# FortuneMU2025/LIDAR_AI_Recommendation_Software

Measured on AMD Instinct MI355X. Metric: M points/sec through SetAbstraction, 65k-pt frames; 1->8 GPU scaling, higher is better.
Workload: dtype f32

## Files before the change

### lidar_ai_recommendation_software_amd/csrc/sa_mlp_x3.hip

```cpp
#include <cmath>
#include <cstdlib>
#include <cstring>
#include <type_traits>
#include <vector>

#include "bq_grid.hpp"
#include "h3.hpp"
#include "sa_shapes.hpp"

namespace {

typedef __bf16 bf16x8 __attribute__((ext_vector_type(8)));
typedef float f32x4 __attribute__((ext_vector_type(4)));
using lidar_h3::f16x8;

__device__ __forceinline__ f32x4 mfma_bf(bf16x8 a, bf16x8 b, f32x4 c)
{
    return __builtin_amdgcn_mfma_f32_16x16x32_bf16(a, b, c, 0, 0, 0);
}
__device__ __forceinline__ f32x4 mfma_bf(f16x8 a, f16x8 b, f32x4 c)
{
    return __builtin_amdgcn_mfma_f32_16x16x32_f16(a, b, c, 0, 0, 0);
}
__device__ __forceinline__ f32x4 mfma_f(float a, float b, f32x4 c)
{
    return __builtin_amdgcn_mfma_f32_16x16x4f32(a, b, c, 0, 0, 0);
}
using lidar::relu_nan;
__device__ __forceinline__ float maxn(float a, float b, float c)
{
    return __builtin_elementwise_maximum(__builtin_elementwise_maximum(a, b), c);
}

__device__ __forceinline__ void split_pair(const f32x4 &t0, const f32x4 &t1, f16x8 &hi, f16x8 &lo, float s)
{
    lidar_h3::split8(t0, t1, s, hi, lo);
}
__device__ __forceinline__ void split_pair(const f32x4 &t0, const f32x4 &t1, bf16x8 &hi, bf16x8 &lo, float)
{
#pragma unroll
    for (int j = 0; j < 8; ++j) {
        const float v = j < 4 ? t0[j] : t1[j - 4];
        const __bf16 h = (__bf16)v;
        hi[j] = h;
        lo[j] = (__bf16)(v - (float)h);
    }
}

template <int C1, int C2, int C3, bool X1 = false>
struct PackX3 {
    static constexpr int T1 = C1 / 16, T2 = C2 / 16, T3 = C3 / 16;
    static constexpr int KS2 = C1 / 32, KS3 = C2 / 32;
    static constexpr int HALVES = X1 ? 1 : 2;
    static constexpr int CH2 = KS2 * 2 * HALVES * 64, CH3 = KS3 * 2 * HALVES * 64;
    static constexpr int W1U4 = T1 * 64 / 4;
};

struct X3Tail {
    int32_t s2, s3;
    float colsum2, bmax2;
};
__device__ __forceinline__ int bound_exp3(const X3Tail &t, int e2)
{
    const float b = (t.colsum2 * ldexpf(1.0f, e2) + t.bmax2) * (1.0f + 0x1p-10f);
    return lidar_h3::exp_of_bits(__float_as_uint(b));
}

enum { L1_XYZ = 0, L1_PRE = 1, L1_PX = 2 };
__device__ __forceinline__ float bf16r(float v) { return (float)(__bf16)v; }

__device__ __forceinline__ float max_row_groups(float v)
{
    const auto a = __builtin_amdgcn_permlane32_swap(__float_as_uint(v), __float_as_uint(v), false, false);
    v = maxn(v, __uint_as_float(a[0]), __uint_as_float(a[1]));
    const auto b = __builtin_amdgcn_permlane16_swap(__float_as_uint(v), __float_as_uint(v), false, false);
    return maxn(v, __uint_as_float(b[0]), __uint_as_float(b[1]));
}

#ifndef LIDAR_BQ_CAP
#define LIDAR_BQ_CAP 512
#endif
#ifndef LIDAR_SA1_W
// ... 203 lines not shown
                        a0[rr][r] = relu_nan(a0[rr][r]);
                        a1[rr][r] = relu_nan(a1[rr][r]);
                    }
                    y2[rr][2 * c < T2 ? 2 * c : 0] = a0[rr];
                    y2[rr][2 * c + 1 < T2 ? 2 * c + 1 : 0] = a1[rr];
                }
                if (c == T2 / 2 - 1) {
#pragma unroll
                    for (int rr = 0; rr < R; ++rr) {
                        float sc = 1.0f;
                        if constexpr (!X1) {
                            e3[rr] = bound_exp3(*reinterpret_cast<const X3Tail *>(Bias + C1 + C2 + C3), e2[rr]);
                            sc = lidar_h3::scale_of(e3[rr]);
                        }
#pragma unroll
                        for (int s = 0; s < KS3; ++s)
                            split_pair(y2[rr][2 * s], y2[rr][2 * s + 1], zh[rr][s], zl[rr][s], sc);
                    }
                }
            } else {
                const int tp = c - T2 / 2;
#pragma unroll
                for (int s = 0; s < KS3; ++s) {
                    const PT h0 = __builtin_bit_cast(PT, wb[((s * 2 + 0) * HV + 0) * 64]);
                    const PT h1 = __builtin_bit_cast(PT, wb[((s * 2 + 1) * HV + 0) * 64]);
                    if constexpr (X1) {
#pragma unroll
                        for (int rr = 0; rr < R; ++rr) {
                            a0[rr] = mfma_bf(zh[rr][s], h0, a0[rr]);
                            a1[rr] = mfma_bf(zh[rr][s], h1, a1[rr]);
                        }
                    } else {
                        const PT l0 = __builtin_bit_cast(PT, wb[((s * 2 + 0) * HV + 1) * 64]);
                        const PT l1 = __builtin_bit_cast(PT, wb[((s * 2 + 1) * HV + 1) * 64]);
#pragma unroll
                        for (int rr = 0; rr < R; ++rr) {
                            a0[rr] = mfma_bf(zh[rr][s], h0, a0[rr]);
                            a1[rr] = mfma_bf(zh[rr][s], h1, a1[rr]);
                            a0[rr] = mfma_bf(zh[rr][s], l0, a0[rr]);
                            a1[rr] = mfma_bf(zh[rr][s], l1, a1[rr]);
                            a0[rr] = mfma_bf(zl[rr][s], h0, a0[rr]);
                            a1[rr] = mfma_bf(zl[rr][s], h1, a1[rr]);
                        }
                    }
                }
#pragma unroll
                for (int hh = 0; hh < 2; ++hh) {
                    const int t = 2 * tp + hh < T3 ? 2 * tp + hh : 0;
                    float v = -INFINITY;
#pragma unroll
                    for (int rr = 0; rr < R; ++rr) {
                        const f32x4 &acc = hh ? a1[rr] : a0[rr];
                        float m4 = maxn(acc[0], acc[1], __builtin_elementwise_maximum(acc[2], acc[3]));
                        if constexpr (!X1) m4 = ldexpf(m4, e3[rr] - 14 - sw3);
                        v = __builtin_elementwise_maximum(v, m4);
                    }
                    v = max_row_groups(v);
                    if (q == (t & 3)) mx[t >> 2] = __builtin_elementwise_maximum(mx[t >> 2], v);
                }
            }
            __syncthreads();
            par ^= 1;
        }
    }
    if (live) {
        float *o = out + unit * out_stride + out_offset;
#pragma unroll
        for (int j = 0; j < T3 / 4; ++j) {
            const int c3 = 16 * (4 * j + q) + col;
            o[c3] = relu_nan(mx[j] + bias_s[C1 + C2 + c3]);
        }
    }
}

#ifndef LIDAR_SA_ABL
#define LIDAR_SA_ABL 0
#endif
#ifndef LIDAR_LEAN_R
#define LIDAR_LEAN_R 2
#endif
#ifndef LIDAR_LEAN_W
#define LIDAR_LEAN_W 4
#endif
template <int C1, int C2, int C3, int NS, bool PFX>
__global__ __launch_bounds__(256, LIDAR_LEAN_W) void sa_x3_lean_kernel(const float *__restrict__ P, int64_t stride,
                                                            const float *__restrict__ Q,
                                                            const int32_t *__restrict__ idx, int n, int m,
                                                            int64_t total, const uint4 *__restrict__ packed,
                                                            float *__restrict__ out, int64_t out_stride,
                                                            int64_t out_offset)
{
    constexpr int R = LIDAR_LEAN_R;
    static_assert(NS % (16 * R) == 0 && C1 % 32 == 0 && C2 % 32 == 0 && C3 % 64 == 0, "tile shapes");
    using K = PackX3<C1, C2, C3, false>;
    constexpr int T2 = K::T2, T3 = K::T3, KS2 = K::KS2, KS3 = K::KS3;
    constexpr int CH2 = K::CH2, CH3 = K::CH3, CHMAX = CH2 > CH3 ? CH2 : CH3;
    constexpr int NL2 = T2 / 2, NL3 = T3 / 2, NSEQ = R * NL2 + NL3;
    constexpr int ITERS = NS / (16 * R);
    constexpr int PER = (CHMAX + 255) / 256;
    static_assert(!PFX || NS % 64 == 0, "PFX: whole 64-row blocks of indices");

    __shared__ uint4 buf0[CHMAX], buf1[CHMAX];
    auto bufp = [&](int p) -> uint4 * { return p ? buf1 : buf0; };
    __shared__ float bias_s[C2 + C3];

    const int tid = threadIdx.x, lane = tid & 63, wave = __builtin_amdgcn_readfirstlane(tid >> 6);
    const int q = lane >> 4, col = lane & 15;
    const int64_t unit = lidar::xcd_block() * 4 + wave;
    const bool live = unit < total;
    const int64_t cc = live ? unit : total - 1;
    const int64_t b = cc / m;

    const uint4 *W2 = packed;
    const uint4 *W3 = W2 + (int64_t)NL2 * CH2;
    const float *Bias = reinterpret_cast<const float *>(W3 + (int64_t)NL3 * CH3);
    const X3Tail tl = *reinterpret_cast<const X3Tail *>(Bias + C1 + C2 + C3);

    auto fetch = [&](int seq, int dst) {
        const int c = (LIDAR_SA_ABL & 1) != 0 ? 0 : seq < R * NL2 ? seq % NL2 : seq - R * NL2 + NL2;
        const uint4 *src = c < NL2 ? W2 + c * CH2 : W3 + (c - NL2) * CH3;
        asm volatile("" : "+s"(src));
        const int len = c < NL2 ? CH2 : CH3;
#pragma unroll
        for (int i = 0; i < PER; ++i) {
            const int base = 256 * i + 64 * wave;
            if ((CH2 == CH3 && CH2 % 256 == 0) || base < len)
                __builtin_amdgcn_global_load_lds((__attribute__((address_space(1))) void *)(src + base + (unsigned)lane),
                                                 (__attribute__((address_space(3))) void *)(&bufp(dst)[base]), 16, 0,
                                                 0);
        }
        __builtin_amdgcn_sched_barrier(0);
    };
    int32_t kall[PFX ? NS / 64 : 1];
    if constexpr (PFX) {
#pragma unroll
        for (int j = 0; j < NS / 64; ++j) kall[j] = idx[cc * NS + 64 * j + lane];
    }
    fetch(0, 0);
    for (int i = tid; i < C2 + C3; i += 256) bias_s[i] = Bias[C1 + i];
    __syncthreads();
    float mx[T3 / 4];
#pragma unroll
    for (int j = 0; j < T3 / 4; ++j) mx[j] = -INFINITY;
    int par = 0;

#pragma unroll 1
    for (int it = 0; it < ITERS; ++it) {
        f16x8 zh[R][KS3], zl[R][KS3];
        int e3[R];
#pragma unroll
        for (int rr = 0; rr < R; ++rr) {
            f16x8 xh[KS2], xl[KS2];
            int e2;
            {
                int zero = 0;
                asm volatile("" : "+v"(zero));
                const int t16 = (it * R + rr) * 16;
                int64_t k;
                if constexpr ((LIDAR_SA_ABL & 4) != 0)
                    k = col;
                else if constexpr (PFX)
                    k = __shfl(kall[t16 >> 6], (t16 & 63) + col, 64);
                else
                    k = idx[cc * NS + t16 + col];
                const f32x4 *pp = reinterpret_cast<const f32x4 *>(P + ((int64_t)b * n + k) * stride + 4 * q);
                const f32x4 *qq = reinterpret_cast<const f32x4 *>(Q + cc * stride + 4 * q + zero);
                f32x4 y[KS2][2];
                uint32_t mb = 0;
#pragma unroll
                for (int s = 0; s < KS2; ++s)
#pragma unroll
                    for (int h = 0; h < 2; ++h) {
                        const f32x4 a = pp[4 * (2 * s + h)], c = qq[4 * (2 * s + h)];
#pragma unroll
                        for (int r = 0; r < 4; ++r) {
                            y[s][h][r] = relu_nan(a[r] - c[r]);
                            mb = max(mb, __float_as_uint(y[s][h][r]));
                        }
                    }
                e2 = lidar_h3::wave_exp(mb);
                const float sc = lidar_h3::scale_of(e2);
#pragma unroll
                for (int s = 0; s < KS2; ++s) split_pair(y[s][0], y[s][1], xh[s], xl[s], sc);
            }
            e3[rr] = bound_exp3(tl, e2);
            const float sc3 = lidar_h3::scale_of(e3[rr]);
#pragma unroll
            for (int c = 0; c < NL2; ++c) {
                fetch(rr * NL2 + c + 1, par ^ 1);
                const uint4 *wb = bufp(par) + lane;
                f32x4 a0 = f32x4{}, a1 = f32x4{};
#pragma unroll
                for (int s = 0; s < KS2; ++s) {
                    const f16x8 h0 = __builtin_bit_cast(f16x8, wb[((s * 2 + 0) * 2 + 0) * 64]);
                    const f16x8 l0 = __builtin_bit_cast(f16x8, wb[((s * 2 + 0) * 2 + 1) * 64]);
                    a0 = mfma_bf(h0, xh[s], a0);
                    a0 = mfma_bf(h0, xl[s], a0);
                    a0 = mfma_bf(l0, xh[s], a0);
                    const f16x8 h1 = __builtin_bit_cast(f16x8, wb[((s * 2 + 1) * 2 + 0) * 64]);
                    const f16x8 l1 = __builtin_bit_cast(f16x8, wb[((s * 2 + 1) * 2 + 1) * 64]);
                    a1 = mfma_bf(h1, xh[s], a1);
                    a1 = mfma_bf(h1, xl[s], a1);
                    a1 = mfma_bf(l1, xh[s], a1);
                }
                const f32x4 b0 = *reinterpret_cast<const f32x4 *>(&bias_s[16 * (2 * c) + 4 * q]);
                const f32x4 b1 = *reinterpret_cast<const f32x4 *>(&bias_s[16 * (2 * c + 1) + 4 * q]);
                const float us = ldexpf(1.0f, e2 - 14 - tl.s2);
#pragma unroll
                for (int r = 0; r < 4; ++r) {
                    a0[r] = relu_nan(fmaf(a0[r], us, b0[r]));
                    a1[r] = relu_nan(fmaf(a1[r], us, b1[r]));
                }
                split_pair(a0, a1, zh[rr][c], zl[rr][c], sc3);
                if constexpr ((LIDAR_SA_ABL & 2) == 0) __syncthreads();
                par ^= 1;
            }
        }
#pragma unroll
        for (int c = 0; c < NL3; ++c) {
            if (c + 1 < NL3 || it + 1 < ITERS) fetch(c + 1 < NL3 ? R * NL2 + c + 1 : 0, par ^ 1);
            const uint4 *wb = bufp(par) + lane;
            f32x4 a0[R], a1[R];
#pragma unroll
            for (int rr = 0; rr < R; ++rr) a0[rr] = a1[rr] = f32x4{};
#pragma unroll
            for (int s = 0; s < KS3; ++s) {
                const f16x8 h0 = __builtin_bit_cast(f16x8, wb[((s * 2 + 0) * 2 + 0) * 64]);
                const f16x8 h1 = __builtin_bit_cast(f16x8, wb[((s * 2 + 1) * 2 + 0) * 64]);
                const f16x8 l0 = __builtin_bit_cast(f16x8, wb[((s * 2 + 0) * 2 + 1) * 64]);
                const f16x8 l1 = __builtin_bit_cast(f16x8, wb[((s * 2 + 1) * 2 + 1) * 64]);
#pragma unroll
                for (int rr = 0; rr < R; ++rr) {
                    a0[rr] = mfma_bf(zh[rr][s], h0, a0[rr]);
                    a1[rr] = mfma_bf(zh[rr][s], h1, a1[rr]);
                    a0[rr] = mfma_bf(zh[rr][s], l0, a0[rr]);
                    a1[rr] = mfma_bf(zh[rr][s], l1, a1[rr]);
                    a0[rr] = mfma_bf(zl[rr][s], h0, a0[rr]);
                    a1[rr] = mfma_bf(zl[rr][s], h1, a1[rr]);
                }
            }
#pragma unroll
            for (int hh = 0; hh < 2; ++hh) {
                const int t = 2 * c + hh;
                float v = -INFINITY;
#pragma unroll
                for (int rr = 0; rr < R; ++rr) {
                    const f32x4 &acc = hh ? a1[rr] : a0[rr];
                    const float m4 = maxn(acc[0], acc[1], __builtin_elementwise_maximum(acc[2], acc[3]));
                    v = __builtin_elementwise_maximum(v, ldexpf(m4, e3[rr] - 14 - tl.s3));
                }
                v = max_row_groups(v);
                if (q == (t & 3)) mx[t >> 2] = __builtin_elementwise_maximum(mx[t >> 2], v);
            }
            if constexpr ((LIDAR_SA_ABL & 2) == 0) __syncthreads();
            par ^= 1;
        }
    }
    static_assert(NSEQ == R * NL2 + NL3, "pass count");
    if (live) {
        float *o = out + unit * out_stride + out_offset;
#pragma unroll
        for (int j = 0; j < T3 / 4; ++j) {
            const int c3 = 16 * (4 * j + q) + col;
            o[c3] = relu_nan(mx[j] + bias_s[C2 + c3]);
        }
    }
}

#ifndef LIDAR_X3_ROWS
#define LIDAR_X3_ROWS 2
#endif
#ifndef LIDAR_X1_ROWS
#define LIDAR_X1_ROWS 2
#endif
template <int NS, bool X1>
constexpr int rows_for()
{
    return X1 && NS >= 16 * LIDAR_X1_ROWS ? LIDAR_X1_ROWS : (NS >= 16 * LIDAR_X3_ROWS ? LIDAR_X3_ROWS : 1);
}

template <int C1, int C2, int C3, int NS, int L1, bool X1 = false, bool LEAN = false>
int launch_x3(const float *p, int64_t stride, const float *q, const int32_t *idx, int64_t batch, int64_t n,
              int64_t m, const void *packed, float *out, int64_t os, int64_t oo, hipStream_t s,
              const float *xyz = nullptr, const float *centres = nullptr)
{
    static_assert(!LEAN || (L1 == L1_PRE && !X1), "the lean kernel: fp32-contract feature levels");
    int64_t total, blocks;
    if (int rc = lidar_sa::launch_geometry("sa_group_mlp_x3", batch, m, 4, total, blocks)) return rc;
    if constexpr (LEAN) {
        hipLaunchKernelGGL((sa_x3_lean_kernel<C1, C2, C3, NS, NS % 64 == 0>), dim3((unsigned)blocks), dim3(256), 0, s,
                           p, stride, q, idx, (int)n, (int)m, total, static_cast<const uint4 *>(packed), out, os, oo);
    } else {
        hipLaunchKernelGGL((sa_x3_kernel<C1, C2, C3, NS, L1, rows_for<NS, X1>(), X1>), dim3((unsigned)blocks),
                           dim3(256), 0, s, p, stride, q, idx, (int)n, (int)m, total,
                           static_cast<const uint4 *>(packed), out, os, oo, xyz, centres, nullptr, 0.0f, 0.0f, nullptr);
    }
    LAUNCH_CHECK();
    return LIDAR_OK;
}

template <int C1, int C2, int C3, int NS, bool XYZ>
int launch_x3_bq(bool x1, const float *xyz, const char *grid, const float *centres, int64_t batch, int64_t n,
                 int64_t m, float radius, const void *packed, float *out, int64_t os, int64_t oo, int32_t *out_idx,
                 hipStream_t s)
{
    if constexpr (XYZ) {
        int64_t total, blocks;
        if (int rc = lidar_sa::launch_geometry("sa_group_mlp_bq", batch, m, 4, total, blocks)) return rc;
        auto go = [&](auto kern) {
            hipLaunchKernelGGL(kern, dim3((unsigned)blocks), dim3(256), 0, s, xyz, (int64_t)3, centres, nullptr, (int)n,
                               (int)m, total, static_cast<const uint4 *>(packed), out, os, oo, nullptr, nullptr, grid,
                               radius, radius * radius, out_idx);
        };
        if (x1)
            go(sa_x3_kernel<C1, C2, C3, NS, L1_XYZ, rows_for<NS, true>(), true, true>);
        else
            go(sa_x3_kernel<C1, C2, C3, NS, L1_XYZ, rows_for<NS, false>(), false, true>);
        LAUNCH_CHECK();
        return LIDAR_OK;
    } else {
        return lidar::fail(LIDAR_EINVAL, "lidar_sa_group_mlp_bq_f32: unsupported (widths, nsample) combination");
    }
}

__host__ uint16_t bf16_rne(float f)
{
    uint32_t u;
    memcpy(&u, &f, 4);
    if ((u & 0x7fffffffu) > 0x7f800000u) return (uint16_t)((u >> 16) | 0x40);
    u += 0x7fffu + ((u >> 16) & 1u);
    return (uint16_t)(u >> 16);
}
__host__ float bf16_to_f(uint16_t h)
{
    const uint32_t u = (uint32_t)h << 16;
    float f;
    memcpy(&f, &u, 4);
    return f;
}
__host__ uint16_t f16_bits(float f)
{
    const _Float16 h = (_Float16)f;
    uint16_t u;
    memcpy(&u, &h, 2);
    return u;
}
__host__ float f16_to_f(uint16_t u)
{
    _Float16 h;
    memcpy(&h, &u, 2);
    return (float)h;
}
__host__ int32_t layer_exp(const float *w, int64_t n)
{
    uint32_t m = 0;
    for (int64_t i = 0; i < n; ++i) {
        uint32_t u;
        memcpy(&u, &w[i], 4);
        m = std::max(m, u & 0x7fffffffu);
    }
    return 14 - lidar_h3::exp_of_bits(m);
}

}

LIDAR_EXPORT int64_t lidar_mlp_packed_size_x3(int32_t xyz_level, int32_t c1, int32_t c2, int32_t c3)
{
    const int64_t w1 = xyz_level ? (int64_t)(c1 / 16) * 64 * 4 : 0;
    return w1 + ((int64_t)(c2 / 32) * (c1 / 32) + (int64_t)(c3 / 32) * (c2 / 32)) * 4 * 64 * 16 +
           (int64_t)(c1 + c2 + c3) * 4 + (int64_t)sizeof(X3Tail);
}

LIDAR_EXPORT int lidar_mlp_pack_x3_f32(int32_t xyz_level, int32_t c1, int32_t c2, int32_t c3, const float *w1,
                                       const float *b1, const float *w2, const float *b2, const float *w3,
// ... 41 lines not shown
        return rc;
    if (batch == 0) return LIDAR_OK;
    ON_DEVICE(h->device);
    hipStream_t s = static_cast<hipStream_t>(stream);
#define LIDAR_SAX3(C1_, C2_, C3_, NS_, X_, LEAN_)                                                              \
    if (!!xyz_level == X_ && c1 == C1_ && c2 == C2_ && c3 == C3_ && nsample == NS_)                            \
        return launch_x3<C1_, C2_, C3_, NS_, X_ ? L1_XYZ : L1_PRE, false, LEAN_>(p, p_stride, q, idx, batch, n, m, \
                                                                                packed, out, out_stride, out_offset, s);
    LIDAR_SA_SHAPES(LIDAR_SAX3)
#undef LIDAR_SAX3
    return lidar::fail(LIDAR_EINVAL, "lidar_sa_group_mlp_x3_f32: unsupported (widths, nsample) combination");
}

LIDAR_EXPORT int64_t lidar_mlp_packed_size_x1(int32_t c1, int32_t c2, int32_t c3)
{
    return (int64_t)(c1 / 16) * 64 * 4 + ((int64_t)(c2 / 32) * (c1 / 32) + (int64_t)(c3 / 32) * (c2 / 32)) * 2 * 64 * 16 +
           (int64_t)(c1 + c2 + c3) * 4;
}

LIDAR_EXPORT int lidar_mlp_pack_x1_f32(int32_t c1, int32_t c2, int32_t c3, const float *w1, const float *b1,
                                       const float *w2, const float *b2, const float *w3, const float *b3,
                                       void *packed)
{
    REQUIRE(w1 && b1 && w2 && b2 && w3 && b3 && packed, "lidar_mlp_pack_x1_f32: null pointer");
    if (int rc = lidar_sa::check_pack_widths("lidar_mlp_pack_x1_f32", c1, c2, c3)) return rc;
    float *f = lidar_sa::write_w1_lanes(static_cast<float *>(packed), w1, c1,
                                        [](float v) { return bf16_to_f(bf16_rne(v)); });
    auto bf = [](float w, int) { return bf16_rne(w); };
    uint16_t *u = reinterpret_cast<uint16_t *>(f);
    u = lidar_sa::write_fragments<1>(u, w2, c1, c2, bf);
    u = lidar_sa::write_fragments<1>(u, w3, c2, c3, bf);
    lidar_sa::write_biases(reinterpret_cast<float *>(u), b1, c1, b2, c2, b3, c3);
    return LIDAR_OK;
}

LIDAR_EXPORT int lidar_sa_group_mlp_x1_f32(lidar_handle *h, int32_t layer1_mode, const float *p, int64_t p_stride,
                                           const float *q, const float *xyz, const float *centres,
                                           const int32_t *idx, int64_t batch, int64_t n, int64_t m, int32_t nsample,
                                           int32_t c1, int32_t c2, int32_t c3, const void *packed, float *out,
                                           int64_t out_stride, int64_t out_offset, void *stream)
{
    REQUIRE(layer1_mode == 0 || layer1_mode == 2, "lidar_sa_group_mlp_x1_f32: layer1_mode must be 0 or 2");
    REQUIRE(layer1_mode == 2 ? (xyz && centres && p_stride >= c1 && p_stride % 4 == 0) : q != nullptr,
            "lidar_sa_group_mlp_x1_f32: mode 0 needs q = centres; mode 2 needs xyz, centres, p_stride >= c1");
    if (int rc = lidar_sa::check_args("lidar_sa_group_mlp_x1_f32", h && p && idx && packed && out,
                                      batch >= 0 && n >= 1 && m >= 1, true, out_offset, c3, out_stride))
        return rc;
    if (batch == 0) return LIDAR_OK;
    ON_DEVICE(h->device);
    hipStream_t s = static_cast<hipStream_t>(stream);
#define LIDAR_SAX1(C1_, C2_, C3_, NS_, X_, LEAN_)                                                                 \
    if (layer1_mode == (X_ ? 0 : 2) && c1 == C1_ && c2 == C2_ && c3 == C3_ && nsample == NS_)                     \
        return launch_x3<C1_, C2_, C3_, NS_, X_ ? L1_XYZ : L1_PX, true>(p, p_stride, X_ ? q : nullptr, idx, batch, n, \
                                                                       m, packed, out, out_stride, out_offset, s, \
                                                                       xyz, centres);
    LIDAR_SA_SHAPES(LIDAR_SAX1)
#undef LIDAR_SAX1
    return lidar::fail(LIDAR_EINVAL, "lidar_sa_group_mlp_x1_f32: unsupported (widths, nsample) combination");
}

LIDAR_EXPORT int lidar_sa_group_mlp_bq_f32(lidar_handle *h, int32_t x1, const float *xyz, const void *grid,
                                           const float *centres, int64_t batch, int64_t n, int64_t m, float radius,
                                           int32_t nsample, int32_t c1, int32_t c2, int32_t c3, const void *packed,
                                           float *out, int64_t out_stride, int64_t out_offset, int32_t *out_idx,
                                           void *stream)
{
    REQUIRE(radius >= 0.0f, "lidar_sa_group_mlp_bq_f32: negative radius");
    if (int rc = lidar_sa::check_args("lidar_sa_group_mlp_bq_f32", h && xyz && grid && centres && packed && out,
                                      batch >= 0 && n >= 1 && n < 0x3fffffff && m >= 1 && m < 0x7fffffff, true,
                                      out_offset, c3, out_stride))
        return rc;
    if (batch == 0) return LIDAR_OK;
    ON_DEVICE(h->device);
    hipStream_t s = static_cast<hipStream_t>(stream);
    const char *g = static_cast<const char *>(grid);
#define LIDAR_SABQ(C1_, C2_, C3_, NS_, X_, LEAN_)                                                              \
    if (X_ && c1 == C1_ && c2 == C2_ && c3 == C3_ && nsample == NS_)                                           \
        return launch_x3_bq<C1_, C2_, C3_, NS_, X_>(x1 != 0, xyz, g, centres, batch, n, m, radius, packed, out, \
                                                    out_stride, out_offset, out_idx, s);
    LIDAR_SA_SHAPES(LIDAR_SABQ)
#undef LIDAR_SABQ
    return lidar::fail(LIDAR_EINVAL, "lidar_sa_group_mlp_bq_f32: unsupported (widths, nsample) combination");
}
```

### lidar_ai_recommendation_software_amd/csrc/bq_grid.hpp

```cpp
#pragma once
#include "common.hpp"

namespace lidar_bq {

constexpr int kTab = 16384;
#ifndef LIDAR_BQ_KCAP
#define LIDAR_BQ_KCAP 512
#endif
constexpr int kCap = LIDAR_BQ_KCAP;
constexpr int kGridMinN = 1024;

struct BqGrid {
    float minx, miny, minz, inv_s;
    int dx, dy, dz, ncell;
    int win_shift, nwin;
    int pad[2];
};

__host__ __device__ constexpr uint64_t grid_frame_bytes(int64_t n)
{
    return 64 + (uint64_t)(kTab + 64) * 4 + (uint64_t)n * 16;
}

__device__ __forceinline__ int cell_of(float v, float lo, float inv_s, int d)
{
    float u = __fmul_rn(__fsub_rn(v, lo), inv_s);
    u = fminf(fmaxf(u, -2.0f), (float)d + 1.0f);
    return (int)floorf(u);
}

__device__ __forceinline__ int point_slot(float x, float y, float z, int k, const BqGrid &g)
{
    const int ix = min(max(cell_of(x, g.minx, g.inv_s, g.dx), 0), g.dx - 1);
    const int iy = min(max(cell_of(y, g.miny, g.inv_s, g.dy), 0), g.dy - 1);
    const int iz = min(max(cell_of(z, g.minz, g.inv_s, g.dz), 0), g.dz - 1);
    return (k >> g.win_shift) * g.ncell + (ix * g.dy + iy) * g.dz + iz;
}

template <class Out>
__device__ __forceinline__ void scan_range(const float *__restrict__ p, int lo, int hi, float cx, float cy,
                                           float cz, float r2, int ns, int lane, uint64_t below, int &cnt,
                                           int &first, Out *o)
{
    for (int k0 = lo; k0 < hi && cnt < ns; k0 += 64) {
        const int k = k0 + lane;
        bool hit = false;
        if (k < hi) hit = lidar::dist2f(p[3 * k], p[3 * k + 1], p[3 * k + 2], cx, cy, cz) < r2;
        const uint64_t mk = __ballot(hit);
        if (mk) {
            if (first < 0) first = k0 + __ffsll((unsigned long long)mk) - 1;
            const int rk = cnt + __popcll(mk & below);
            if (hit && rk < ns) o[rk] = k;
            cnt += __popcll(mk);
        }
    }
}

__device__ __forceinline__ void lds_wave_sync()
{
    asm volatile("s_waitcnt lgkmcnt(0)" ::: "memory");
    __builtin_amdgcn_wave_barrier();
}

template <int CAP, class Out, bool BM = true>
__device__ __forceinline__ void grid_query_wave(const float *__restrict__ p, const char *__restrict__ fw, int n,
                                                float cx, float cy, float cz, float r, float r2, int ns,
                                                int lane, int *hw, Out *o)
{
    const BqGrid g = *reinterpret_cast<const BqGrid *>(fw);
    const int *tab = reinterpret_cast<const int *>(fw + 64);
    const float4 *sp = reinterpret_cast<const float4 *>(fw + 64 + (kTab + 64) * 4);
    const uint64_t below = (1ull << lane) - 1;

    const float delta = __fadd_rn(__fmul_rn(__fmul_rn(r, g.inv_s), 1.0f + 1.0f / 1024.0f), 1.0f / 1024.0f);
    const float ux = __fmul_rn(__fsub_rn(cx, g.minx), g.inv_s), uy = __fmul_rn(__fsub_rn(cy, g.miny), g.inv_s),
                uz = __fmul_rn(__fsub_rn(cz, g.minz), g.inv_s);
    auto lo_of = [](float u, float dl, int d) {
        return max((int)floorf(fminf(fmaxf(__fsub_rn(u, dl), -2.0f), (float)d + 1.0f)), 0);
    };
    auto hi_of = [](float u, float dl, int d) {
        return min((int)floorf(fminf(fmaxf(__fadd_rn(u, dl), -2.0f), (float)d + 1.0f)), d - 1);
    };
    const int lox = lo_of(ux, delta, g.dx), hix = hi_of(ux, delta, g.dx);
    const int loy = lo_of(uy, delta, g.dy), hiy = hi_of(uy, delta, g.dy);
    const int loz = lo_of(uz, delta, g.dz), hiz = hi_of(uz, delta, g.dz);
    int cnt = 0, first = -1;
    const bool full = (hix - lox) > 2 || (hiy - loy) > 2;
    const int jx = lox + lane / 3, jy = loy + lane % 3;
    const bool col_ok = !full && lane < 9 && jx <= hix && jy <= hiy && loz <= hiz;
    const int colbase = (jx * g.dy + jy) * g.dz + loz;
    int st = 0, len = 0;
    if (col_ok && g.nwin > 0) {
        st = tab[colbase];
        len = tab[colbase + (hiz - loz) + 1] - st;
    }
    const bool bitmap = BM && ns >= 64 && !full && ((int64_t)1 << g.win_shift) <= 32 * (int64_t)CAP;
    unsigned long long *bm = reinterpret_cast<unsigned long long *>(hw);
    for (int win = 0; win < g.nwin && cnt < ns; ++win) {
        const int wlo = win << g.win_shift, whi = min(n, (win + 1) << g.win_shift);
        const int cst = st, clen = len;
        if (col_ok && win + 1 < g.nwin) {
            const int s1 = (win + 1) * g.ncell + colbase;
            st = tab[s1];
            len = tab[s1 + (hiz - loz) + 1] - st;
        }
        const int incl = lidar::row_incl_scan_i32(clen);
        const int tot = full ? CAP + 1 : __builtin_amdgcn_readlane(incl, 8);
        if (tot == 0) continue;
        if (!bitmap && tot > CAP) {
            scan_range(p, wlo, whi, cx, cy, cz, r2, ns, lane, below, cnt, first, o);
            continue;
        }
        const int nwords = (whi - wlo + 63) >> 6;
        if (bitmap) {
            for (int i = lane; i < nwords; i += 64) bm[i] = 0ull;
            lds_wave_sync();
        }
        const int excl = incl - clen;
        int e[9], s[9];
#pragma unroll
        for (int j = 0; j < 9; ++j) {
            e[j] = __builtin_amdgcn_readlane(excl, j);
            s[j] = __builtin_amdgcn_readlane(cst, j);
        }
        int hc = 0;
        for (int t0 = 0; t0 < tot; t0 += 256) {
            float4 qv[4];
#pragma unroll
            for (int u = 0; u < 4; ++u) {
                const int t = t0 + 64 * u + lane;
                int pos = s[0] + t;
#pragma unroll
                for (int j = 1; j < 9; ++j)
                    if (t >= e[j]) pos = s[j] + (t - e[j]);
                qv[u] = t < tot ? sp[pos] : make_float4(0.f, 0.f, 0.f, 0.f);
            }
#pragma unroll
            for (int u = 0; u < 4; ++u) {
                const int t = t0 + 64 * u + lane;
                const bool hit = t < tot && lidar::dist2f(qv[u].x, qv[u].y, qv[u].z, cx, cy, cz) < r2;
                const uint64_t mk = __ballot(hit);
                if (hit) {
                    if (bitmap) {
                        const int o1 = __float_as_int(qv[u].w) - wlo;
                        atomicOr(&bm[o1 >> 6], 1ull << (o1 & 63));
                    } else {
                        hw[hc + __popcll(mk & below)] = __float_as_int(qv[u].w);
                    }
                }
                hc += __popcll(mk);
            }
        }
        if (hc == 0) continue;
        if (bitmap) {
            lds_wave_sync();
            int base = 0, mnv = 0x7fffffff;
            for (int c0 = 0; c0 < nwords && cnt + base < ns; c0 += 64) {
                const int wi = c0 + lane;
                unsigned long long wd = wi < nwords ? bm[wi] : 0ull;
                const int pc = __popcll(wd);
                const int ex = lidar::wave_incl_scan_i32(pc) - pc;
                if (wd) mnv = min(mnv, wlo + 64 * wi + (int)__ffsll(wd) - 1);
                int rk = cnt + base + ex;
                while (wd && rk < ns) {
                    const int j = __ffsll(wd) - 1;
                    o[rk++] = wlo + 64 * wi + j;
                    wd &= wd - 1;
                }
                base += __builtin_amdgcn_readlane(ex + pc, 63);
            }
            if (first < 0) first = (int)lidar::wave_min_u32_dpp((uint32_t)mnv);
            cnt += hc;
            lds_wave_sync();
            continue;
        }
        if (lane < 4) hw[hc + lane] = 0x7fffffff;
        lds_wave_sync();
        int mnv = 0x7fffffff;
        for (int e0 = 0; e0 < hc; e0 += 64) {
            const int ei = e0 + lane;
            const int v = ei < hc ? hw[ei] : 0x7fffffff;
            int rank = 0;
            for (int i = 0; i < hc; i += 4) {
                const int4 h4 = *reinterpret_cast<const int4 *>(hw + i);
                rank += (h4.x < v) + (h4.y < v) + (h4.z < v) + (h4.w < v);
            }
            if (ei < hc && cnt + rank < ns) o[cnt + rank] = v;
            mnv = min(mnv, v);
        }
        if (first < 0) first = (int)lidar::wave_min_u32_dpp((uint32_t)mnv);
        cnt += hc;
        lds_wave_sync();
    }
    const int fill = first < 0 ? 0 : first;
    for (int s2 = min(cnt, ns) + lane; s2 < ns; s2 += 64) o[s2] = fill;
}

}
```

Baseline: 1269.

## Add prefetching lean SA kernel that overlaps next-row gathers with MLP passes

Adds a new lean set-abstraction kernel, on by default, that DMAs the neighbour indices and the centre feature row into LDS up front. It prefetches the next 16-row gather of point features into registers, spread across the layer-2 and layer-3 MFMA passes, and uses vmcnt-counted pass ends so the barrier waits only for the weight chunk and not the in-flight row loads. The aim is to hide gather latency behind matrix work. In exchange it uses more LDS and registers, which may reduce occupancy, and it depends on exact load counting for correctness. It also adds optional per-phase s_memtime instrumentation behind LIDAR_DIAG.

```diff
diff --git a/lidar_ai_recommendation_software_amd/csrc/sa_mlp_x3.hip b/lidar_ai_recommendation_software_amd/csrc/sa_mlp_x3.hip
--- a/lidar_ai_recommendation_software_amd/csrc/sa_mlp_x3.hip
+++ b/lidar_ai_recommendation_software_amd/csrc/sa_mlp_x3.hip
@@ -1,3 +1,4 @@
+#include <atomic>
 #include <cmath>
 #include <cstdlib>
 #include <cstring>
@@ -367,13 +368,64 @@
 #ifndef LIDAR_LEAN_W
 #define LIDAR_LEAN_W 4
 #endif
+#ifndef LIDAR_LEAN_PF
+#define LIDAR_LEAN_PF 1
+#endif
+
+enum { PH_PRO = 0, PH_GATHER, PH_L1, PH_BODY, PH_END, PH_EPI, PH_N };
+#ifdef LIDAR_DIAG
+struct LeanClock {
+    uint32_t t, acc[PH_N];
+    __device__ __forceinline__ uint32_t now()
+    {
+        uint64_t v;
+        __builtin_amdgcn_sched_barrier(0);
+        asm volatile("s_memtime %0\n\ts_waitcnt lgkmcnt(0)" : "=s"(v)::"memory");
+        __builtin_amdgcn_sched_barrier(0);
+        return (uint32_t)v;
+    }
+    __device__ __forceinline__ void start()
+    {
+#pragma unroll
+        for (int k = 0; k < PH_N; ++k) acc[k] = 0;
+        t = now();
+    }
+    __device__ __forceinline__ void lap(int k)
+    {
+        const uint32_t v = now();
+        acc[k] += v - t;
+        t = v;
+    }
+    __device__ __forceinline__ void landed(int k)
+    {
+        asm volatile("s_waitcnt vmcnt(0)" ::: "memory");
+        lap(k);
+    }
+    __device__ __forceinline__ void store(uint64_t *diag, int64_t wave_id, int lane, int centres)
+    {
+        if (diag != nullptr && lane == 0) {
+#pragma unroll
+            for (int k = 0; k < PH_N; ++k) diag[wave_id * 8 + k] = acc[k];
+            diag[wave_id * 8 + 6] = (uint64_t)centres;
+            diag[wave_id * 8 + 7] = 0;
+        }
+    }
+};
+#define LEAN_DIAG(...) __VA_ARGS__
+uint64_t *g_sa2_rec = nullptr;
+int64_t g_sa2_rec_cap = 0;
+std::atomic<int64_t> g_sa2_rec_used{0};
+#else
+#define LEAN_DIAG(...)
+#endif
+
 template <int C1, int C2, int C3, int NS, bool PFX>
 __global__ __launch_bounds__(256, LIDAR_LEAN_W) void sa_x3_lean_kernel(const float *__restrict__ P, int64_t stride,
                                                             const float *__restrict__ Q,
                                                             const int32_t *__restrict__ idx, int n, int m,
                                                             int64_t total, const uint4 *__restrict__ packed,
                                                             float *__restrict__ out, int64_t out_stride,
-                                                            int64_t out_offset)
+                                                            int64_t out_offset, uint64_t *__restrict__ diag)
 {
     constexpr int R = LIDAR_LEAN_R;
     static_assert(NS % (16 * R) == 0 && C1 % 32 == 0 && C2 % 32 == 0 && C3 % 64 == 0, "tile shapes");
@@ -395,6 +447,7 @@
     const bool live = unit < total;
     const int64_t cc = live ? unit : total - 1;
     const int64_t b = cc / m;
+    LEAN_DIAG(LeanClock clk; clk.start();)
 
     const uint4 *W2 = packed;
     const uint4 *W3 = W2 + (int64_t)NL2 * CH2;
@@ -428,6 +481,7 @@
 #pragma unroll
     for (int j = 0; j < T3 / 4; ++j) mx[j] = -INFINITY;
     int par = 0;
+    LEAN_DIAG(clk.lap(PH_PRO);)
 
 #pragma unroll 1
     for (int it = 0; it < ITERS; ++it) {
@@ -452,11 +506,23 @@
                 const f32x4 *qq = reinterpret_cast<const f32x4 *>(Q + cc * stride + 4 * q + zero);
                 f32x4 y[KS2][2];
                 uint32_t mb = 0;
+#ifdef LIDAR_DIAG
+                f32x4 pr[KS2][2], qr[KS2][2];
 #pragma unroll
                 for (int s = 0; s < KS2; ++s)
 #pragma unroll
+                    for (int h = 0; h < 2; ++h) pr[s][h] = pp[4 * (2 * s + h)], qr[s][h] = qq[4 * (2 * s + h)];
+                clk.landed(PH_GATHER);
+#endif
+#pragma unroll
+                for (int s = 0; s < KS2; ++s)
+#pragma unroll
                     for (int h = 0; h < 2; ++h) {
+#ifdef LIDAR_DIAG
+                        const f32x4 a = pr[s][h], c = qr[s][h];
+#else
                         const f32x4 a = pp[4 * (2 * s + h)], c = qq[4 * (2 * s + h)];
+#endif
 #pragma unroll
                         for (int r = 0; r < 4; ++r) {
                             y[s][h][r] = relu_nan(a[r] - c[r]);
@@ -470,6 +536,7 @@
             }
             e3[rr] = bound_exp3(tl, e2);
             const float sc3 = lidar_h3::scale_of(e3[rr]);
+            LEAN_DIAG(clk.lap(PH_L1);)
 #pragma unroll
             for (int c = 0; c < NL2; ++c) {
                 fetch(rr * NL2 + c + 1, par ^ 1);
@@ -497,7 +564,9 @@
                     a1[r] = relu_nan(fmaf(a1[r], us, b1[r]));
                 }
                 split_pair(a0, a1, zh[rr][c], zl[rr][c], sc3);
+                LEAN_DIAG(clk.lap(PH_BODY);)
                 if constexpr ((LIDAR_SA_ABL & 2) == 0) __syncthreads();
+                LEAN_DIAG(clk.lap(PH_END);)
                 par ^= 1;
             }
         }
@@ -537,7 +606,9 @@
                 v = max_row_groups(v);
                 if (q == (t & 3)) mx[t >> 2] = __builtin_elementwise_maximum(mx[t >> 2], v);
             }
+            LEAN_DIAG(clk.lap(PH_BODY);)
             if constexpr ((LIDAR_SA_ABL & 2) == 0) __syncthreads();
+            LEAN_DIAG(clk.lap(PH_END);)
             par ^= 1;
         }
     }
@@ -550,6 +621,237 @@
             o[c3] = relu_nan(mx[j] + bias_s[C2 + c3]);
         }
     }
+    LEAN_DIAG(clk.landed(PH_EPI); clk.store(diag, lidar::xcd_block() * 4 + wave, lane, 1);)
+}
+
+template <int N>
+__device__ __forceinline__ void pass_end()
+{
+    static_assert(N >= 0 && N < 16, "vmcnt's low four bits");
+    __builtin_amdgcn_s_waitcnt(0x0070 | N);
+    asm volatile("s_barrier" ::: "memory");
+}
+
+template <int C1, int C2, int C3, int NS>
+__global__ __launch_bounds__(256, LIDAR_LEAN_W) void sa_x3_lean_pf_kernel(const float *__restrict__ P, int64_t stride,
+                                                            const float *__restrict__ Q,
+                                                            const int32_t *__restrict__ idx, int n, int m,
+                                                            int64_t total, const uint4 *__restrict__ packed,
+                                                            float *__restrict__ out, int64_t out_stride,
+                                                            int64_t out_offset, uint64_t *__restrict__ diag)
+{
+    constexpr int R = 2;
+    using K = PackX3<C1, C2, C3, false>;
+    constexpr int T3 = K::T3, KS2 = K::KS2, KS3 = K::KS3;
+    constexpr int CH = K::CH2, NL2 = K::T2 / 2, NL3 = T3 / 2, PER = CH / 256;
+    constexpr int ITERS = NS / (16 * R);
+    constexpr int NP = 2 * KS2;
+    constexpr int PF2 = NP / NL2;
+    constexpr int PF3 = NP / KS3;
+    static_assert(K::CH2 == K::CH3 && CH % 256 == 0, "equal whole chunks: the pass ends count the loads behind them");
+    static_assert(NP % NL2 == 0 && NP % KS3 == 0 && NP < 16, "the row prefetch spreads over the passes");
+    static_assert(NS % 64 == 0 && C1 % 64 == 0 && C3 % 64 == 0, "whole 64-word DMAs of indices and of the Q row");
+
+    __shared__ uint4 buf0[CH], buf1[CH];
+    auto bufp = [&](int p) -> uint4 * { return p ? buf1 : buf0; };
+    __shared__ float bias_s[C2 + C3];
+    __shared__ float q_s[4][C1];
+    __shared__ int32_t k_s[4][NS];
+
+    const int tid = threadIdx.x, lane = tid & 63, wave = __builtin_amdgcn_readfirstlane(tid >> 6);
+    const int q = lane >> 4, col = lane & 15;
+    const int64_t unit = lidar::xcd_block() * 4 + wave;
+    const bool live = unit < total;
+    const int64_t cc = live ? unit : total - 1;
+    const int64_t b = cc / m;
+    LEAN_DIAG(LeanClock clk; clk.start();)
+
+    const uint4 *W2 = packed;
+    const uint4 *W3 = W2 + (int64_t)NL2 * CH;
+    const float *Bias = reinterpret_cast<const float *>(W3 + (int64_t)NL3 * CH);
+    const X3Tail tl = *reinterpret_cast<const X3Tail *>(Bias + C1 + C2 + C3);
+
+    auto fetch = [&](int seq, int dst) {
+        const int c = seq < R * NL2 ? seq % NL2 : seq - R * NL2 + NL2;
+        const uint4 *src = W2 + c * CH;
+        asm volatile("" : "+s"(src));
+#pragma unroll
+        for (int i = 0; i < PER; ++i) {
+            const int base = 256 * i + 64 * wave;
+            __builtin_amdgcn_global_load_lds((__attribute__((address_space(1))) void *)(src + base + (unsigned)lane),
+                                             (__attribute__((address_space(3))) void *)(&bufp(dst)[base]), 16, 0, 0);
+        }
+        __builtin_amdgcn_sched_barrier(0);
+    };
+    {
+        const int32_t *ks = idx + cc * NS;
+        const float *qs = Q + cc * stride;
+        asm volatile("" : "+s"(ks), "+s"(qs));
+#pragma unroll
+        for (int j = 0; j < NS / 64; ++j)
+            __builtin_amdgcn_global_load_lds((const __attribute__((address_space(1))) void *)(ks + 64 * j + (unsigned)lane),
+                                             (__attribute__((address_space(3))) void *)(&k_s[wave][64 * j]), 4, 0, 0);
+#pragma unroll
+        for (int j = 0; j < C1 / 64; ++j)
+            __builtin_amdgcn_global_load_lds((const __attribute__((address_space(1))) void *)(qs + 64 * j + (unsigned)lane),
+                                             (__attribute__((address_space(3))) void *)(&q_s[wave][64 * j]), 4, 0, 0);
+    }
+    auto rows = [&](int t16) {
+        const int64_t k = k_s[wave][t16 + col];
+        const float *frame = P + b * n * stride;
+        return reinterpret_cast<const f32x4 *>(frame + (k * stride + 4 * q));
+    };
+
+    fetch(0, 0);
+    for (int i = tid; i < C2 + C3; i += 256) bias_s[i] = Bias[C1 + i];
+    pass_end<0>();
+    f32x4 pre[NP];
+    {
+        const f32x4 *pp = rows(0);
+#pragma unroll
+        for (int j = 0; j < NP; ++j) pre[j] = pp[4 * j];
+    }
+    float mx[T3 / 4];
+#pragma unroll
+    for (int j = 0; j < T3 / 4; ++j) mx[j] = -INFINITY;
+    int par = 0;
+    LEAN_DIAG(clk.lap(PH_PRO);)
+
+#pragma unroll 1
+    for (int it = 0; it < ITERS; ++it) {
+        const bool lastit = it + 1 == ITERS;
+        f16x8 zh[R][KS3], zl[R][KS3];
+        int e3[R];
+#pragma unroll
+        for (int rr = 0; rr < R; ++rr) {
+            f16x8 xh[KS2], xl[KS2];
+            int e2;
+            {
+                LEAN_DIAG(clk.landed(PH_GATHER);)
+                f32x4 y[KS2][2];
+                uint32_t mb = 0;
+#pragma unroll
+                for (int s = 0; s < KS2; ++s)
+#pragma unroll
+                    for (int h = 0; h < 2; ++h) {
+                        const f32x4 a = pre[2 * s + h];
+                        const f32x4 c = *reinterpret_cast<const f32x4 *>(&q_s[wave][16 * (2 * s + h) + 4 * q]);
+#pragma unroll
+                        for (int r = 0; r < 4; ++r) {
+                            y[s][h][r] = relu_nan(a[r] - c[r]);
+                            mb = max(mb, __float_as_uint(y[s][h][r]));
+                        }
+                    }
+                e2 = lidar_h3::wave_exp(mb);
+                const float sc = lidar_h3::scale_of(e2);
+#pragma unroll
+                for (int s = 0; s < KS2; ++s) split_pair(y[s][0], y[s][1], xh[s], xl[s], sc);
+            }
+            e3[rr] = bound_exp3(tl, e2);
+            const float sc3 = lidar_h3::scale_of(e3[rr]);
+            LEAN_DIAG(clk.lap(PH_L1);)
+            const f32x4 *pp = rr == 0 ? rows((it * R + 1) * 16) : nullptr;
+#pragma unroll
+            for (int c = 0; c < NL2; ++c) {
+                fetch(rr * NL2 + c + 1, par ^ 1);
+                if (rr == 0) {
+#pragma unroll
+                    for (int j = c * PF2; j < (c + 1) * PF2; ++j) pre[j] = pp[4 * j];
+                    __builtin_amdgcn_sched_barrier(0);
+                }
+                const uint4 *wb = bufp(par) + lane;
+                f32x4 a0 = f32x4{}, a1 = f32x4{};
+#pragma unroll
+                for (int s = 0; s < KS2; ++s) {
+                    const f16x8 h0 = __builtin_bit_cast(f16x8, wb[((s * 2 + 0) * 2 + 0) * 64]);
+                    const f16x8 l0 = __builtin_bit_cast(f16x8, wb[((s * 2 + 0) * 2 + 1) * 64]);
+                    a0 = mfma_bf(h0, xh[s], a0);
+                    a0 = mfma_bf(h0, xl[s], a0);
+                    a0 = mfma_bf(l0, xh[s], a0);
+                    const f16x8 h1 = __builtin_bit_cast(f16x8, wb[((s * 2 + 1) * 2 + 0) * 64]);
+                    const f16x8 l1 = __builtin_bit_cast(f16x8, wb[((s * 2 + 1) * 2 + 1) * 64]);
+                    a1 = mfma_bf(h1, xh[s], a1);
+                    a1 = mfma_bf(h1, xl[s], a1);
+                    a1 = mfma_bf(l1, xh[s], a1);
+                }
+                const f32x4 b0 = *reinterpret_cast<const f32x4 *>(&bias_s[16 * (2 * c) + 4 * q]);
+                const f32x4 b1 = *reinterpret_cast<const f32x4 *>(&bias_s[16 * (2 * c + 1) + 4 * q]);
+                const float us = ldexpf(1.0f, e2 - 14 - tl.s2);
+#pragma unroll
+                for (int r = 0; r < 4; ++r) {
+                    a0[r] = relu_nan(fmaf(a0[r], us, b0[r]));
+                    a1[r] = relu_nan(fmaf(a1[r], us, b1[r]));
+                }
+                split_pair(a0, a1, zh[rr][c], zl[rr][c], sc3);
+                LEAN_DIAG(clk.lap(PH_BODY);)
+                if (rr == 0)
+                    pass_end<PF2>();
+                else
+                    pass_end<0>();
+                LEAN_DIAG(clk.lap(PH_END);)
+                par ^= 1;
+            }
+        }
+        const f32x4 *pp = rows(lastit ? 0 : (it + 1) * R * 16);
+#pragma unroll
+        for (int c = 0; c < NL3; ++c) {
+            if (c + 1 < NL3 || !lastit) fetch(c + 1 < NL3 ? R * NL2 + c + 1 : 0, par ^ 1);
+            const uint4 *wb = bufp(par) + lane;
+            f32x4 a0[R], a1[R];
+#pragma unroll
+            for (int rr = 0; rr < R; ++rr) a0[rr] = a1[rr] = f32x4{};
+#pragma unroll
+            for (int s = 0; s < KS3; ++s) {
+                const f16x8 h0 = __builtin_bit_cast(f16x8, wb[((s * 2 + 0) * 2 + 0) * 64]);
+                const f16x8 h1 = __builtin_bit_cast(f16x8, wb[((s * 2 + 1) * 2 + 0) * 64]);
+                const f16x8 l0 = __builtin_bit_cast(f16x8, wb[((s * 2 + 0) * 2 + 1) * 64]);
+                const f16x8 l1 = __builtin_bit_cast(f16x8, wb[((s * 2 + 1) * 2 + 1) * 64]);
+#pragma unroll
+                for (int rr = 0; rr < R; ++rr) {
+                    a0[rr] = mfma_bf(zh[rr][s], h0, a0[rr]);
+                    a1[rr] = mfma_bf(zh[rr][s], h1, a1[rr]);
+                    a0[rr] = mfma_bf(zh[rr][s], l0, a0[rr]);
+                    a1[rr] = mfma_bf(zh[rr][s], l1, a1[rr]);
+                    a0[rr] = mfma_bf(zl[rr][s], h0, a0[rr]);
+                    a1[rr] = mfma_bf(zl[rr][s], h1, a1[rr]);
+                }
+                if (c == NL3 - 1) {
+#pragma unroll
+                    for (int j = s * PF3; j < (s + 1) * PF3; ++j) pre[j] = pp[4 * j];
+                }
+            }
+#pragma unroll
+            for (int hh = 0; hh < 2; ++hh) {
+                const int t = 2 * c + hh;
+                float v = -INFINITY;
+#pragma unroll
+                for (int rr = 0; rr < R; ++rr) {
+                    const f32x4 &acc = hh ? a1[rr] : a0[rr];
+                    const float m4 = maxn(acc[0], acc[1], __builtin_elementwise_maximum(acc[2], acc[3]));
+                    v = __builtin_elementwise_maximum(v, ldexpf(m4, e3[rr] - 14 - tl.s3));
+                }
+                v = max_row_groups(v);
+                if (q == (t & 3)) mx[t >> 2] = __builtin_elementwise_maximum(mx[t >> 2], v);
+            }
+            LEAN_DIAG(clk.lap(PH_BODY);)
+            if (c == NL3 - 1)
+                pass_end<NP>();
+            else
+                pass_end<0>();
+            LEAN_DIAG(clk.lap(PH_END);)
+            par ^= 1;
+        }
+    }
+    if (live) {
+        float *o = out + unit * out_stride + out_offset;
+#pragma unroll
+        for (int j = 0; j < T3 / 4; ++j) {
+            const int c3 = 16 * (4 * j + q) + col;
+            o[c3] = relu_nan(mx[j] + bias_s[C2 + c3]);
+        }
+    }
+    __builtin_amdgcn_s_waitcnt(0x0070);
+    LEAN_DIAG(clk.lap(PH_EPI); clk.store(diag, unit, lane, 1);)
 }
 
 #ifndef LIDAR_X3_ROWS
@@ -570,11 +872,25 @@
               const float *xyz = nullptr, const float *centres = nullptr)
 {
     static_assert(!LEAN || (L1 == L1_PRE && !X1), "the lean kernel: fp32-contract feature levels");
+    static_assert(LIDAR_SA_ABL == 0 || LIDAR_LEAN_PF == 0, "the ablations are sa_x3_lean_kernel's");
     int64_t total, blocks;
     if (int rc = lidar_sa::launch_geometry("sa_group_mlp_x3", batch, m, 4, total, blocks)) return rc;
     if constexpr (LEAN) {
-        hipLaunchKernelGGL((sa_x3_lean_kernel<C1, C2, C3, NS, NS % 64 == 0>), dim3((unsigned)blocks), dim3(256), 0, s,
-                           p, stride, q, idx, (int)n, (int)m, total, static_cast<const uint4 *>(packed), out, os, oo);
+        uint64_t *diag = nullptr;
+#ifdef LIDAR_DIAG
+        if (g_sa2_rec) {
+            const int64_t need = blocks * 4 * 8, off = g_sa2_rec_used.fetch_add(need);
+            if (off + need <= g_sa2_rec_cap) diag = g_sa2_rec + off;
+        }
+#endif
+        auto go = [&](auto kern) {
+            hipLaunchKernelGGL(kern, dim3((unsigned)blocks), dim3(256), 0, s, p, stride, q, idx, (int)n, (int)m, total,
+                               static_cast<const uint4 *>(packed), out, os, oo, diag);
+        };
+        if constexpr (LIDAR_LEAN_PF != 0)
+            go(sa_x3_lean_pf_kernel<C1, C2, C3, NS>);
+        else
+            go(sa_x3_lean_kernel<C1, C2, C3, NS, NS % 64 == 0>);
     } else {
         hipLaunchKernelGGL((sa_x3_kernel<C1, C2, C3, NS, L1, rows_for<NS, X1>(), X1>), dim3((unsigned)blocks),
                            dim3(256), 0, s, p, stride, q, idx, (int)n, (int)m, total,
@@ -782,3 +1098,14 @@
 #undef LIDAR_SABQ
     return lidar::fail(LIDAR_EINVAL, "lidar_sa_group_mlp_bq_f32: unsupported (widths, nsample) combination");
 }
+
+#ifdef LIDAR_DIAG
+LIDAR_EXPORT int lidar_diag_sa2_record(uint64_t *buf, int64_t cap_words)
+{
+    g_sa2_rec = buf;
+    g_sa2_rec_cap = buf ? cap_words : 0;
+    g_sa2_rec_used = 0;
+    return LIDAR_OK;
+}
+LIDAR_EXPORT int64_t lidar_diag_sa2_recorded(void) { return std::min<int64_t>(g_sa2_rec_used, g_sa2_rec_cap); }
+#endif
```

Result: no change. 1265 (-0.3%).

## Trim grid column z-runs to the query sphere and assign lanes per column

Applied to the files above, without the earlier changes.

Each of the nine candidate grid columns now computes a z-range trimmed by the sphere's horizontal gap to that column, so fewer cells' points are loaded and tested. The gather loop gives seven lanes to each column and walks the column directly. This replaces the prefix-scan plus nine-way position search and the per-window total-count readlane. It also swaps correctly rounded intrinsics for plain float ops and uses mbcnt for ranking. Risks include lane underuse when columns are uneven, more loop iterations for long columns, and subtle boundary differences from the trimming math.

```diff
diff --git a/lidar_ai_recommendation_software_amd/csrc/bq_grid.hpp b/lidar_ai_recommendation_software_amd/csrc/bq_grid.hpp
--- a/lidar_ai_recommendation_software_amd/csrc/bq_grid.hpp
+++ b/lidar_ai_recommendation_software_amd/csrc/bq_grid.hpp
@@ -22,12 +22,51 @@
     return 64 + (uint64_t)(kTab + 64) * 4 + (uint64_t)n * 16;
 }
 
-__device__ __forceinline__ int cell_of(float v, float lo, float inv_s, int d)
-{
-    float u = __fmul_rn(__fsub_rn(v, lo), inv_s);
+
+__host__ __device__ inline int cell_of(float v, float lo, float inv_s, int d)
+{
+    float u = (v - lo) * inv_s;
     u = fminf(fmaxf(u, -2.0f), (float)d + 1.0f);
     return (int)floorf(u);
 }
+
+__host__ __device__ inline float query_delta(float r, float inv_s)
+{
+    return r * inv_s * (1.0f + 1.0f / 1024.0f) + 1.0f / 1024.0f;
+}
+__host__ __device__ inline int cell_lo(float u, float dl, int d)
+{
+    return max((int)floorf(fminf(fmaxf(u - dl, -2.0f), (float)d + 1.0f)), 0);
+}
+__host__ __device__ inline int cell_hi(float u, float dl, int d)
+{
+    return min((int)floorf(fminf(fmaxf(u + dl, -2.0f), (float)d + 1.0f)), d - 1);
+}
+
+__host__ __device__ inline void column_zrun(float ux, float uy, float uz, float delta, int jx, int jy, int dx, int dy,
+                                            int dz, int loz, int hiz, bool trim, int &zlo, int &zhi)
+{
+    zlo = loz;
+    zhi = hiz;
+    if (!trim) return;
+    const float gx = fmaxf(fmaxf(jx > 0 ? (float)jx - ux : 0.0f, jx < dx - 1 ? ux - (float)(jx + 1) : 0.0f), 0.0f);
+    const float gy = fmaxf(fmaxf(jy > 0 ? (float)jy - uy : 0.0f, jy < dy - 1 ? uy - (float)(jy + 1) : 0.0f), 0.0f);
+    const float d2 = delta * delta;
+    const float h2 = (d2 - (gx * gx + gy * gy)) + d2 * (1.0f / 65536.0f);
+    if (h2 <= 0.0f) {
+        zlo = 1;
+        zhi = 0;
+        return;
+    }
+#ifdef __HIP_DEVICE_COMPILE__
+    const float zr = __builtin_amdgcn_sqrtf(h2) + 1.0f / 4096.0f;
+#else
+    const float zr = sqrtf(h2) + 1.0f / 4096.0f;
+#endif
+    zlo = max(cell_lo(uz, zr, dz), loz);
+    zhi = min(cell_hi(uz, zr, dz), hiz);
+}
+constexpr float kTrimMinR = 9.094947e-13f;
 
 __device__ __forceinline__ int point_slot(float x, float y, float z, int k, const BqGrid &g)
 {
@@ -72,27 +111,24 @@
     const float4 *sp = reinterpret_cast<const float4 *>(fw + 64 + (kTab + 64) * 4);
     const uint64_t below = (1ull << lane) - 1;
 
-    const float delta = __fadd_rn(__fmul_rn(__fmul_rn(r, g.inv_s), 1.0f + 1.0f / 1024.0f), 1.0f / 1024.0f);
-    const float ux = __fmul_rn(__fsub_rn(cx, g.minx), g.inv_s), uy = __fmul_rn(__fsub_rn(cy, g.miny), g.inv_s),
-                uz = __fmul_rn(__fsub_rn(cz, g.minz), g.inv_s);
-    auto lo_of = [](float u, float dl, int d) {
-        return max((int)floorf(fminf(fmaxf(__fsub_rn(u, dl), -2.0f), (float)d + 1.0f)), 0);
-    };
-    auto hi_of = [](float u, float dl, int d) {
-        return min((int)floorf(fminf(fmaxf(__fadd_rn(u, dl), -2.0f), (float)d + 1.0f)), d - 1);
-    };
-    const int lox = lo_of(ux, delta, g.dx), hix = hi_of(ux, delta, g.dx);
-    const int loy = lo_of(uy, delta, g.dy), hiy = hi_of(uy, delta, g.dy);
-    const int loz = lo_of(uz, delta, g.dz), hiz = hi_of(uz, delta, g.dz);
+    const float delta = query_delta(r, g.inv_s);
+    const float ux = (cx - g.minx) * g.inv_s, uy = (cy - g.miny) * g.inv_s, uz = (cz - g.minz) * g.inv_s;
+    const int lox = cell_lo(ux, delta, g.dx), hix = cell_hi(ux, delta, g.dx);
+    const int loy = cell_lo(uy, delta, g.dy), hiy = cell_hi(uy, delta, g.dy);
+    const int loz = cell_lo(uz, delta, g.dz), hiz = cell_hi(uz, delta, g.dz);
     int cnt = 0, first = -1;
+    constexpr int kColLanes = 7;
     const bool full = (hix - lox) > 2 || (hiy - loy) > 2;
-    const int jx = lox + lane / 3, jy = loy + lane % 3;
-    const bool col_ok = !full && lane < 9 && jx <= hix && jy <= hiy && loz <= hiz;
-    const int colbase = (jx * g.dy + jy) * g.dz + loz;
+    const int col = lane / kColLanes, cw = lane - col * kColLanes;
+    const int jx = lox + col / 3, jy = loy + col % 3;
+    int zlo, zhi;
+    column_zrun(ux, uy, uz, delta, jx, jy, g.dx, g.dy, g.dz, loz, hiz, r >= kTrimMinR, zlo, zhi);
+    const bool col_ok = !full && col < 9 && jx <= hix && jy <= hiy && zlo <= zhi;
+    const int colbase = (jx * g.dy + jy) * g.dz + zlo, run = zhi - zlo + 1;
     int st = 0, len = 0;
     if (col_ok && g.nwin > 0) {
         st = tab[colbase];
-        len = tab[colbase + (hiz - loz) + 1] - st;
+        len = tab[colbase + run] - st;
     }
     const bool bitmap = BM && ns >= 64 && !full && ((int64_t)1 << g.win_shift) <= 32 * (int64_t)CAP;
     unsigned long long *bm = reinterpret_cast<unsigned long long *>(hw);
@@ -102,12 +138,15 @@
         if (col_ok && win + 1 < g.nwin) {
             const int s1 = (win + 1) * g.ncell + colbase;
             st = tab[s1];
-            len = tab[s1 + (hiz - loz) + 1] - st;
-        }
-        const int incl = lidar::row_incl_scan_i32(clen);
-        const int tot = full ? CAP + 1 : __builtin_amdgcn_readlane(incl, 8);
-        if (tot == 0) continue;
-        if (!bitmap && tot > CAP) {
+            len = tab[s1 + run] - st;
+        }
+        bool over = full;
+        if (!full) {
+            if (__ballot(clen > 0) == 0) continue;
+            if (!bitmap && __ballot(clen > CAP / 9) != 0)
+                over = __builtin_amdgcn_readlane(lidar::wave_incl_scan_i32(cw == 0 ? clen : 0), 63) > CAP;
+        }
+        if (!bitmap && over) {
             scan_range(p, wlo, whi, cx, cy, cz, r2, ns, lane, below, cnt, first, o);
             continue;
         }
@@ -116,36 +155,29 @@
             for (int i = lane; i < nwords; i += 64) bm[i] = 0ull;
             lds_wave_sync();
         }
-        const int excl = incl - clen;
-        int e[9], s[9];
-#pragma unroll
-        for (int j = 0; j < 9; ++j) {
-            e[j] = __builtin_amdgcn_readlane(excl, j);
-            s[j] = __builtin_amdgcn_readlane(cst, j);
-        }
         int hc = 0;
-        for (int t0 = 0; t0 < tot; t0 += 256) {
+        for (int k0 = cw; __ballot(k0 < clen) != 0; k0 += 4 * kColLanes) {
             float4 qv[4];
+            uint64_t in_run[4];
 #pragma unroll
             for (int u = 0; u < 4; ++u) {
-                const int t = t0 + 64 * u + lane;
-                int pos = s[0] + t;
-#pragma unroll
-                for (int j = 1; j < 9; ++j)
-                    if (t >= e[j]) pos = s[j] + (t - e[j]);
-                qv[u] = t < tot ? sp[pos] : make_float4(0.f, 0.f, 0.f, 0.f);
-            }
+                const int k = k0 + kColLanes * u;
+                in_run[u] = __ballot(k < clen);
+                qv[u] = sp[min((unsigned)(cst + k), (unsigned)(n - 1))];
+            }
+            asm volatile("" : "+v"(qv[0].w));
 #pragma unroll
             for (int u = 0; u < 4; ++u) {
-                const int t = t0 + 64 * u + lane;
-                const bool hit = t < tot && lidar::dist2f(qv[u].x, qv[u].y, qv[u].z, cx, cy, cz) < r2;
-                const uint64_t mk = __ballot(hit);
-                if (hit) {
+                if (u > 0 && !in_run[u]) continue;
+                const bool near = lidar::dist2f(qv[u].x, qv[u].y, qv[u].z, cx, cy, cz) < r2;
+                const uint64_t mk = __ballot(near) & in_run[u];
+                if (near && k0 + kColLanes * u < clen) {
                     if (bitmap) {
                         const int o1 = __float_as_int(qv[u].w) - wlo;
                         atomicOr(&bm[o1 >> 6], 1ull << (o1 & 63));
                     } else {
-                        hw[hc + __popcll(mk & below)] = __float_as_int(qv[u].w);
+                        (hw + hc)[__builtin_amdgcn_mbcnt_hi((uint32_t)(mk >> 32), __builtin_amdgcn_mbcnt_lo((uint32_t)mk, 0))] =
+                            __float_as_int(qv[u].w);
                     }
                 }
                 hc += __popcll(mk);
```

Result: no change. 1280 before, 1279 after, median of 2 (-0.1%).
